# OthmanB/TAMCMC-C

Hardware: AMD Instinct MI355X
Metric: MCMC samples/sec (whole node), 1e5 nu-bins x 100 params x 20 tempered chains (higher is better)
Workload: dtype f64

## Files before the change

### tamcmc-c_amd/csrc/dev_sampler.hip

```cpp
#include <hip/hip_runtime.h>

#include <atomic>
#include <chrono>
#include <hip/hip_ext.h>

#include <cmath>
#include <cstdio>
#include <cstdlib>
#include <cstring>
#include <algorithm>
#include <type_traits>
#include <utility>
#include <vector>

#include "ctx.h"
#include "rgb_prestep.h"
#include "dev_sampler.h"
#include "kernels.h"
#include "loglike_tile.h"
#include "dev_unpack.h"
#include "fd_batch.h"
#include "mode_tables.h"
#include "rng.h"
#include "step_schedule.h"
// ... 189 lines not shown
    double *d_pr, *d_ex, *d_T;
    DCHK(I.dalloc(&d_pl, 11)); DCHK(I.dalloc(&d_idx, Nv)); DCHK(I.dalloc(&d_sw, Np));
    DCHK(I.dalloc(&d_pr, 4 * Np)); DCHK(I.dalloc(&d_ex, 10)); DCHK(I.dalloc(&d_T, C));
    DCHK(up(d_pl, in.plength, 11, st)); DCHK(up(d_idx, in.index_to_relax, Nv, st)); DCHK(up(d_sw, in.priors_switch, Np, st));
    DCHK(up(d_pr, in.priors, 4 * Np, st)); DCHK(up(d_ex, in.extra_priors, 10, st)); DCHK(up(d_T, in.Tcoefs, C, st));
    a.desc.plength = d_pl; a.index_to_relax = d_idx; a.desc.priors_switch = d_sw; a.desc.priors = d_pr; a.desc.extra = d_ex; a.Tcoefs = d_T;
    DCHK(I.dalloc(&a.vars_cur, 2 * C * Nv)); DCHK(I.dalloc(&a.params_cur, 2 * C * Np));
    DCHK(I.dalloc(&a.vars_prop, 2 * CD * Nv)); DCHK(I.dalloc(&a.params_prop, 2 * CD * Np));
    DCHK(I.dalloc(&a.logL_cur, 2 * C)); DCHK(I.dalloc(&a.logPr_cur, 2 * C)); DCHK(I.dalloc(&a.logPost_cur, 2 * C));
    DCHK(I.dalloc(&a.init_logL, C)); DCHK(I.dalloc(&a.logPr_prop, 2 * CD)); DCHK(I.dalloc(&a.status_prop, 2 * CD));
    DCHK(I.dalloc(&a.Pmove, C)); DCHK(I.dalloc(&a.moved, C)); DCHK(I.dalloc(&a.counters, 8 + C + 64));
    a.grad_cur = nullptr; a.gradP_cur = nullptr;
    if (I.use_drift) {
        DCHK(I.dalloc(&a.grad_cur, 2 * C * Nv)); DCHK(I.dalloc(&a.gradP_cur, 2 * C * Nv));
        DCHK(I.dalloc(&I.mala.grad_prop, C * Nv)); DCHK(I.dalloc(&I.mala.gradP_prop, C * Nv)); DCHK(I.dalloc(&I.mala.drift_cur, C * Nv));
        DCHK(I.dalloc(&I.mala.out, C * 5));
    }
    DCHK(I.dalloc(&a.lz, 2 * C * Nv)); DCHK(I.dalloc(&a.LT, C * Nv * Nv)); DCHK(I.dalloc(&a.cov, C * Nv * Nv)); DCHK(I.dalloc(&a.mu, C * Nv)); DCHK(I.dalloc(&a.sigma, C));
    DCHK(I.dalloc(&a.mults, CD * (size_t)a.desc.per + 1)); DCHK(I.dalloc(&a.pairs, 2 * CD)); DCHK(I.dalloc(&a.nh, CD)); DCHK(I.dalloc(&a.nn, CD));
    DCHK(I.dalloc(&a.noise, CD * (size_t)a.desc.stride));
    DCHK(hipMemsetAsync(a.counters, 0, (8 + C + 64) * sizeof(long), st));
    DCHK(hipMemsetAsync(a.moved, 0, C * sizeof(int), st));
    DCHK(hipMemsetAsync(a.Pmove, 0, C * sizeof(double), st));
    a.samples = nullptr; a.stats = nullptr;
    I.lds_base = (Np + 2 * Nv + 1) * sizeof(double) + unpack_lds_bytes() + 32;
    I.lds_adapt = (Nv * Nv + Nv) * sizeof(double);
    a.chol_in_lds = (I.lds_base + I.lds_adapt <= 150 * 1024) ? 1 : 0;
    if (!a.chol_in_lds) { DCHK(I.dalloc(&I.adapt_scratch, C * (Nv * Nv + Nv))); I.lds_adapt = 0; }
    if (I.lds_base + I.lds_adapt > 64 * 1024) {
        DCHK(hipFuncSetAttribute((const void *)k_iterate<true>, hipFuncAttributeMaxDynamicSharedMemorySize, (int)(I.lds_base + I.lds_adapt)));
        DCHK(hipFuncSetAttribute((const void *)k_iterate<false>, hipFuncAttributeMaxDynamicSharedMemorySize, (int)(I.lds_base + I.lds_adapt)));
    }
    mt::PolyTab *d_tab;
    DCHK(I.dalloc(&d_tab, 1));
    hipLaunchKernelGGL(k_fill_poly, dim3(1), dim3(64), 0, st, d_tab);
    DCHK(hipGetLastError());
    a.desc.poly = d_tab;
    for (int i = 0; i < 64; i++) { DCHK(hipEventCreate(&I.ev[i][0])); DCHK(hipEventCreate(&I.ev[i][1])); I.n_ev = i + 1; }
    for (int i = 0; i < 8; i++) { DCHK(hipEventCreate(&I.gev[i][0])); DCHK(hipEventCreate(&I.gev[i][1])); I.n_gev = i + 1; }
    {
        const int G = I.G;
        I.gst[0] = st;
        for (int g = 1; g < G; g++) DCHK(hipStreamCreateWithFlags(&I.gst[g], hipStreamNonBlocking));
        DCHK(hipEventCreateWithFlags(&I.ev_fork, hipEventDisableTiming));
        for (int g = 0; g < 4; g++) {
            DCHK(hipEventCreateWithFlags(&I.ev_kb[g], hipEventDisableTiming));
            DCHK(hipEventCreateWithFlags(&I.ev_ki[g], hipEventDisableTiming));
            DCHK(hipEventCreateWithFlags(&I.ev_join[g], hipEventDisableTiming));
        }
        I.ev_made = true;
    }
    {
        FusedArgs &f = I.f;
        f.NS = 2 * in.C + 8;
        {
            const int h = (int)(((long)in.C * 1) / 2);
            f.xsplit = (I.G == 2 && h >= 3 && in.C - h >= 3) ? h : in.C;
        }
        const size_t NS = (size_t)f.NS;
        DCHK(I.dalloc(&f.cand_vars, 3 * NS * Nv)); DCHK(I.dalloc(&f.cand_params, 3 * NS * Np)); DCHK(I.dalloc(&f.cand_logPr, 6 * NS));
        DCHK(I.dalloc(&f.cand_stP, 6 * NS)); DCHK(I.dalloc(&f.cand_stR, 3 * NS)); DCHK(I.dalloc(&f.cand_rej, 3 * NS));
        DCHK(I.dalloc(&f.mults, 3 * NS * (size_t)a.desc.per + 1)); DCHK(I.dalloc(&f.pairs, 6 * NS)); DCHK(I.dalloc(&f.nh, 3 * NS)); DCHK(I.dalloc(&f.nn, 3 * NS));
        DCHK(I.dalloc(&f.noise, 3 * NS * (size_t)a.desc.stride));
        DCHK(I.dalloc(&f.slot, 2 * C)); DCHK(I.dalloc(&f.prop_logPr, 2 * C)); DCHK(I.dalloc(&f.prop_st, 2 * C)); DCHK(I.dalloc(&f.quick, 2 * C * QN)); DCHK(I.dalloc(&f.lz, 2 * C * Nv));
        DCHK(I.dalloc(&f.qcount, 2));
        DCHK(hipMemsetAsync(f.qcount, 0, 2 * sizeof(unsigned long long), st));
        f.qmargin = 1e-11;
        DCHK(hipMemsetAsync(f.nn, 0, 3 * NS * sizeof(int), st));
        DCHK(hipMemsetAsync(f.cand_stP, 0, 6 * NS * sizeof(int), st));
        DCHK(hipMemsetAsync(f.cand_rej, 0, 3 * NS * sizeof(int), st));
        DCHK(hipMemsetAsync(f.cand_stR, 0, 3 * NS * sizeof(int), st));
        f.part = nullptr;
        f.psum = nullptr;
        f.bg = nullptr;
        const size_t role_lds = (Np + 2 * Nv + 1) * sizeof(double) + unpack_lds_bytes() + 32;
        I.fused_ok = !I.rgb && role_lds <= sizeof(tile::TileLds<tile::M_FAST_DIRECT, 64>);
    }
    DCHK(hipStreamSynchronize(st));
    return TAMCMC_OK;
}

int DevSampler::download_gradient(double *grad, double *grad_prior) {
    Impl &I = *impl;
    tamcmc_hip_ctx *c = I.ctx;
    if (!I.use_drift || !I.a.grad_cur || !I.grad_valid) return TAMCMC_ERR_BAD_ARG;
    DCHK(hipSetDevice(c->device));
    const size_t n = (size_t)I.a.C * I.a.Nv;
    DCHK(hipStreamSynchronize(c->stream));
    if (grad) DCHK(hipMemcpy(grad, I.a.grad_cur + (size_t)I.parity * n, n * sizeof(double), hipMemcpyDeviceToHost));
    if (grad_prior) DCHK(hipMemcpy(grad_prior, I.a.gradP_cur + (size_t)I.parity * n, n * sizeof(double), hipMemcpyDeviceToHost));
    return TAMCMC_OK;
}

int DevSampler::download_last_proposal(double *vars_prop, double *grad_prop) {
    Impl &I = *impl;
    tamcmc_hip_ctx *c = I.ctx;
    if (!I.use_drift) return TAMCMC_ERR_BAD_ARG;
    DCHK(hipSetDevice(c->device));
    const size_t n = (size_t)I.a.C * I.a.Nv;
    DCHK(hipStreamSynchronize(c->stream));
    if (vars_prop) DCHK(hipMemcpy(vars_prop, I.a.vars_prop, n * sizeof(double), hipMemcpyDeviceToHost));
    if (grad_prop) DCHK(hipMemcpy(grad_prop, I.mala.grad_prop, n * sizeof(double), hipMemcpyDeviceToHost));
    return TAMCMC_OK;
}

void DevSampler::info(long out[11]) const {
    const Impl &I = *impl;
    unsigned long long qc[2] = {0, 0};
    if (I.f.qcount && hipSetDevice(I.ctx->device) == hipSuccess) (void)hipMemcpy(qc, I.f.qcount, sizeof qc, hipMemcpyDeviceToHost);
    out[8] = I.n_stretch; out[9] = (long)qc[0]; out[10] = (long)qc[1];
// ... 129 lines not shown
static const bool g_call_timeline = getenv("TAMCMC_CALL_TIMELINE") != nullptr;
struct CallTimeline {
    std::chrono::steady_clock::time_point t[5];
    int n = 0;
    void mark() { if (g_call_timeline && n < 5) t[n++] = std::chrono::steady_clock::now(); }
    ~CallTimeline() {
        if (!g_call_timeline || n < 2) return;
        fprintf(stderr, "run() timeline (us):");
        for (int k = 1; k < n; k++) fprintf(stderr, " %.1f", std::chrono::duration<double, std::micro>(t[k] - t[k - 1]).count());
        fprintf(stderr, "\n");
    }
};

struct DevSampler::Impl::KernelTiming {
    Impl &I;
    tamcmc_hip_ctx *c;
    int used_ev = 0;
    std::vector<std::pair<int, long>> fused_ev;
    int g_used = 0;
    long g_launches = 0, g_iters = 0;
    double kernel_ms = 0;
    long n_launch = 0, n_eval = 0;
    bool stretch_timed = false;
    int fe = 0;
    long next_sample = 0;

    hipEvent_t *lockstep_pair(long k, long every) { return c->timing && k % every == 0 && used_ev < I.n_ev - 16 ? I.ev[used_ev++] : nullptr; }
    int drain_events(double launches_represented, long evals) {
        if (used_ev) {
            double tot = 0;
            for (int e = 0; e < used_ev; e++) {
                float ms = 0;
                DCHK(hipEventElapsedTime(&ms, I.ev[e][0], I.ev[e][1]));
                tot += ms;
            }
            kernel_ms += tot / used_ev * launches_represented;
            n_launch += (long)launches_represented;
            n_eval += evals;
        }
        used_ev = 0;
        return TAMCMC_OK;
    }
    void begin_fused(long len) {
        stretch_timed = c->timing && fused_ev.size() < 16;
        fe = I.n_ev - 1 - (int)fused_ev.size();
        next_sample = len >= 97 ? 48 : len / 2;
    }
    hipEvent_t *stretch_pair() { return stretch_timed ? I.ev[fe] : nullptr; }
    hipEvent_t *sampled_pair(long k) {
        if (!(stretch_timed && g_used < I.n_gev && k >= next_sample)) return nullptr;
        next_sample += 97;
        return I.gev[g_used++];
    }
    void end_fused(long len, bool split, long n_split) {
        if (!stretch_timed) return;
        if (!split) fused_ev.push_back({fe, len});
        else { g_launches += 2 * n_split + (len - n_split); g_iters += len; }
    }
    int total() {
        for (const auto &e : fused_ev) {
            float ms = 0;
            DCHK(hipEventElapsedTime(&ms, I.ev[e.first][0], I.ev[e.first][1]));
            kernel_ms += ms;
            n_launch += e.second;
            n_eval += e.second * (long)I.a.C;
        }
        if (g_launches > 0) {
            double tot = 0;
            for (int e = 0; e < g_used; e++) {
                float ms = 0;
                DCHK(hipEventElapsedTime(&ms, I.gev[e][0], I.gev[e][1]));
                tot += ms;
            }
            if (g_used > 0) {
                kernel_ms += tot / g_used * (double)g_launches;
                n_launch += g_launches;
                n_eval += g_iters * (long)I.a.C;
            }
        }
        c->kernel_ms += kernel_ms;
        c->launches += n_launch;
        c->evals += n_eval;
        return TAMCMC_OK;
    }
};

static hipError_t copy_records(double *samples, double *stats, const DevSamplerArgs &a, size_t n_iter, hipStream_t st) {
    const size_t C = (size_t)a.C, Nv = (size_t)a.Nv;
    hipError_t e = hipSuccess;
    if (samples) e = hipMemcpyAsync(samples, a.samples, n_iter * C * Nv * 8, hipMemcpyDeviceToHost, st);
    if (stats && e == hipSuccess) e = hipMemcpyAsync(stats, a.stats, n_iter * C * 3 * 8, hipMemcpyDeviceToHost, st);
    return e;
}

struct DevSampler::Impl::RunCall {
    Impl &I;
    tamcmc_hip_ctx *c;
    DevSamplerArgs &a;
    const long it0, n_iter;
    const char *learn;
    double *samples, *stats;
    hipStream_t st;
    CallTimeline &tl;
    KernelTiming T;
    DevSamplerArgs args;
    LoglikeArgs la[4], lf[3];
    int goff[5];
    double *zc_smp = nullptr, *zc_st = nullptr;
    bool use_fused = false;
    bool split_ok = false;
    int P;
    StepCtl sc{};
    int q = 0;
    bool s1_must_wait = false;
    bool s1_ahead = false;
    bool s1_open = false;

    RunCall(Impl &I_, CallTimeline &tl_, long it0_, long n_iter_, const char *learn_, double *samples_, double *stats_)
        : I(I_), c(I_.ctx), a(I_.a), it0(it0_), n_iter(n_iter_), learn(learn_), samples(samples_), stats(stats_), st(I_.ctx->stream),
          tl(tl_), T{I_, I_.ctx}, P(I_.parity) {}

    int prepare() {
        const size_t C = (size_t)a.C, Nv = (size_t)a.Nv;
        const int tb = tile_bins(c->wgs, c->K);
        a.ntiles = (a.desc.Nx + tb - 1) / tb;
        DCHK(c->d_part.reserve(C * (size_t)a.ntiles * 2));
        a.partials = c->d_part.p;
        a.tile_bins = tb;
        a.bg = nullptr;
        use_fused = I.fused_ok && c->step_scheme != 1 && c->wgs == 64 && (c->K == 4 || c->K == 8 || c->K == 16);
        I.f.qmargin = c->quick_decide == 1 ? (double)INFINITY : 1e-11;
        const size_t NS = (size_t)I.f.NS;
        I.f.bg = nullptr;
        if (c->precision == TAMCMC_PRECISION_FAST) {
            DCHK(c->d_bg.reserve(C * (size_t)a.ntiles * 8));
            a.bg = c->d_bg.p;
            if (use_fused) {
                DCHK(I.fused_bg.reserve(3 * NS * (size_t)a.ntiles * 8));
                I.f.bg = I.fused_bg.p;
            }
        }
        if (use_fused) {
            DCHK(I.fused_part.reserve(2 * C * (size_t)a.ntiles * 2));
            I.f.part = I.fused_part.p;
            DCHK(I.fused_psum.reserve(2 * C * (size_t)a.ntiles));
            I.f.psum = I.fused_psum.p;
        }
        split_ok = I.f.xsplit < a.C && c->step_scheme != 2 && (c->step_scheme == 3 || (long)a.C * a.ntiles >= 2500);
        auto grown = [](size_t need, size_t have, size_t unit) { const size_t floor_ = 256 * unit; return std::max(std::max(need, floor_), have * 2); };
        zc_smp = I.device_view(samples, (size_t)n_iter * C * Nv * 8);
        zc_st = I.device_view(stats, (size_t)n_iter * C * 3 * 8);
        if (samples && !zc_smp && I.smp_cap < (size_t)n_iter * C * Nv) {
            const size_t cap = grown((size_t)n_iter * C * Nv, I.smp_cap, C * Nv);
            DCHK(I.dalloc(&a.samples, cap));
            I.smp_cap = cap;
        }
        if (stats && !zc_st && I.stat_cap < (size_t)n_iter * C * 3) {
            const size_t cap = grown((size_t)n_iter * C * 3, I.stat_cap, C * 3);
            DCHK(I.dalloc(&a.stats, cap));
            I.stat_cap = cap;
        }
        args = a;
        args.samples = samples ? (zc_smp ? zc_smp : a.samples) : nullptr;
        args.stats = stats ? (zc_st ? zc_st : a.stats) : nullptr;
        const int G = I.G;
        for (int g = 0; g <= G; g++) goff[g] = (int)(((long)a.C * g) / G);
        auto fill_common = [&](LoglikeArgs &l, int B) {
            l.x = c->dx.p; l.y = c->dy.p; l.logx = c->dlogx.p; l.Nx = a.desc.Nx; l.B = B; l.ntiles = a.ntiles;
            l.x0 = a.desc.x_first; l.step = a.desc.step; l.noise_stride = a.desc.stride; l.model = nullptr; l.tile_rot = I.tile_rot;
        };
        for (int g = 0; g < G; g++) {
            LoglikeArgs &l = la[g];
            const int first = goff[g];
            fill_common(l, goff[g + 1] - goff[g]);
            l.mults = a.mults; l.offsets = a.pairs + 2 * first; l.noise = a.noise + (size_t)first * a.desc.stride;
            l.per = a.desc.per; l.slot0 = first;
            l.nharvey = a.nh + first; l.nnoise = a.nn + first; l.partials = a.partials + (size_t)first * a.ntiles * 2;
            l.bg_poly = a.bg ? a.bg + (size_t)first * a.ntiles * 8 : nullptr;
        }
        for (int e = 0; e < 3; e++) {
            LoglikeArgs &l = lf[e];
            const FusedArgs &f = I.f;
            fill_common(l, a.C);
            l.mults = f.mults + (size_t)e * NS * a.desc.per; l.offsets = f.pairs + (size_t)e * 2 * NS; l.noise = f.noise + (size_t)e * NS * a.desc.stride;
            l.nharvey = f.nh + (size_t)e * NS; l.nnoise = f.nn + (size_t)e * NS; l.partials = f.part;
            l.bg_poly = f.bg ? f.bg + (size_t)e * NS * a.ntiles * 8 : nullptr;
            l.per = a.desc.per; l.slot0 = 0;
        }
        return TAMCMC_OK;
    }

    int swap_pair_of(long it) const { return swap_pair(a.seed, a.C, a.dN_mixing, it, nullptr); }

    int run_lockstep(long ia, long ib) {
        const int G = I.G;
        const size_t C = (size_t)a.C;
        I.armed_it = -1;
        I.it_lockstep += ib - ia;
        if (G > 1) {
            DCHK(hipEventRecord(I.ev_fork, st));
            for (int g = 1; g < G; g++) DCHK(hipStreamWaitEvent(I.gst[g], I.ev_fork, 0));
// ... 37 lines not shown
            }
            P ^= 1;
            pending = 1;
            if (i < ib && I.rgb) {
                RgbDeviceTables R;
                R.mults = a.mults; R.pairs = a.pairs; R.nh = a.nh; R.nn = a.nn; R.noise = a.noise; R.stride = a.desc.stride;
                R.status = a.status_prop + (size_t)P * C;
                R.bg = a.bg; R.ntiles = a.ntiles; R.tile_bins = a.tile_bins;
                for (int g = 0; g < G; g++) {
                    int rc = rgb_device_stage(c, goff[g], goff[g + 1] - goff[g], I.rgb_bmax, g, a.desc.per, R, I.gst[g]);
                    if (rc) return rc;
                }
            }
            if (i < ib) {
                for (int g = 0; g < G; g++) {
                    hipEvent_t *pair = g == 0 ? T.lockstep_pair(i - ia, ev_every) : nullptr;
                    if (pair) DCHK(hipEventRecord(pair[0], I.gst[g]));
                    DCHK(launch_loglike(la[g], c->precision, c->wgs, c->K, false, I.gst[g]));
                    if (pair) DCHK(hipEventRecord(pair[1], I.gst[g]));
                }
            }
        }
        for (int g = 1; g < G; g++) {
            DCHK(hipEventRecord(I.ev_join[g], I.gst[g]));
            DCHK(hipStreamWaitEvent(st, I.ev_join[g], 0));
        }
        if (c->timing) {
            DCHK(hipStreamSynchronize(st));
            return T.drain_events((double)len * G, len * (long)a.C);
        }
        return TAMCMC_OK;
    }

    int sync_arg_image() {
        const size_t n1 = (sizeof(DevSamplerArgs) + 15) & ~(size_t)15, n2 = sizeof(FusedArgs);
        std::vector<unsigned char> img(n1 + n2, 0);
        std::memcpy(img.data(), &args, sizeof(DevSamplerArgs));
        std::memcpy(img.data() + n1, &I.f, sizeof(FusedArgs));
        if (!I.d_argcopy) DCHK(I.dalloc(&I.d_argcopy, n1 + n2));
        if (img != I.h_argcopy) {
            DCHK(hipMemcpyAsync(I.d_argcopy, img.data(), n1 + n2, hipMemcpyHostToDevice, st));
            DCHK(hipStreamSynchronize(st));
            I.h_argcopy = img;
            I.armed_it = -1;
        }
        sc.ga = (const DevSamplerArgs *)I.d_argcopy;
        sc.gf = (const FusedArgs *)(I.d_argcopy + n1);
        return TAMCMC_OK;
    }

    int fused_entry(long ia, bool *launched) {
        *launched = !(I.armed_it == it0 + ia && I.armed_q == q);
        if (!*launched) return TAMCMC_OK;
        const int nbr = 8 * I.f.NS;
        const int nlz2 = ((2 * a.C + 7) / 8) * 8;
        sc.it = it0 + ia; sc.rec = -1; sc.q = q; sc.flags = ST_LZ; sc.nbr = 0; sc.nlz = nlz2; sc.n_lz_live = 2 * a.C; sc.it_lz = it0 + ia; sc.q_lz = q;
        DCHK(launch_step(c->precision, c->K, nlz2, st, args, I.f, lf[0], sc));
        sc.flags = ST_ENTRY; sc.nbr = nbr; sc.nlz = 0; sc.n_lz_live = 0;
        DCHK(launch_step(c->precision, c->K, nbr, st, args, I.f, lf[0], sc));
        return TAMCMC_OK;
    }

    int launch_group(int first, int cnt, int A, int A_prev, long i, bool settled, hipStream_t stream, hipEvent_t *ev = nullptr) {
        const bool owns_pair = A >= first && A + 1 < first + cnt;
        const int ntiles_pad = ((a.ntiles + 7) / 8) * 8;
        sc.it = it0 + i; sc.rec = ((samples || stats) && !settled) ? i - 1 : (long)-1; sc.q = q;
        sc.flags = ST_L | ST_BR | ST_LZ | ST_COMMIT | (settled ? ST_FIRST : 0);
#ifdef TAMCMC_PROBE
        if (const char *ep = getenv("TAMCMC_PROBE_STEP")) {
            const int pm = atoi(ep);
            if (pm & 1) sc.flags &= ~ST_BR;
            if (pm & 2) sc.flags &= ~ST_COMMIT;
            if (pm & 4) sc.flags &= ~ST_LZ;
            if (pm & 8) sc.flags |= ST_FIRST;
            if (pm & 16) sc.flags &= ~ST_L;
        }
#endif
        sc.first = first; sc.cnt = cnt; sc.extra = owns_pair ? 1 : 0; sc.pairA = settled ? -1 : A_prev;
        sc.nbr = 8 * (2 * cnt + (owns_pair ? 4 : 0)); sc.nlz = ((2 * cnt + 7) / 8) * 8; sc.n_lz_live = cnt; sc.it_lz = it0 + i + 2; sc.q_lz = q;
        LoglikeArgs lq = lf[(it0 + i) % 3];
        lq.B = cnt;
        lq.partials = I.f.part + ((size_t)q * a.C + first) * a.ntiles * 2;
        DCHK(launch_step(c->precision, c->K, sc.nbr + sc.nlz + ntiles_pad * cnt, stream, args, I.f, lq, sc, ev ? ev[0] : nullptr, ev ? ev[1] : nullptr));
        return TAMCMC_OK;
    }

    int launch_close(int first, int cnt, long ib, hipStream_t stream) {
        sc.it = it0 + ib; sc.rec = (samples || stats) ? ib - 1 : (long)-1; sc.q = q;
        sc.flags = ST_COMMIT;
        sc.first = first; sc.cnt = cnt; sc.extra = 0;
        sc.nbr = 0; sc.nlz = ((cnt + 7) / 8) * 8; sc.n_lz_live = 0; sc.it_lz = 0; sc.q_lz = 0;
        DCHK(launch_step(c->precision, c->K, sc.nlz, stream, args, I.f, lf[0], sc));
        return TAMCMC_OK;
    }

    int s1_waits_for_st() {
        DCHK(hipEventRecord(I.ev_fork, st));
        DCHK(hipStreamWaitEvent(I.gst[1], I.ev_fork, 0));
        return TAMCMC_OK;
    }
    int st_waits_for_s1() {
        DCHK(hipEventRecord(I.ev_join[1], I.gst[1]));
        DCHK(hipStreamWaitEvent(st, I.ev_join[1], 0));
        return TAMCMC_OK;
    }

    int run_fused(long ia, long ib) {
        const long len = ib - ia;
        const int first1 = I.f.xsplit;
        hipStream_t s1 = I.gst[1];
        I.it_fused += len;
        I.n_stretch += 1;
        q = P;
        sc = StepCtl{};
        if (int rc = sync_arg_image()) return rc;
        sc.first = 0; sc.cnt = a.C; sc.extra = 1;
        bool entered;
        if (int rc = fused_entry(ia, &entered)) return rc;
        s1_must_wait = ia > 0 || entered;
        s1_ahead = false;
        T.begin_fused(len);
        if (!split_ok && T.stretch_pair()) DCHK(hipEventRecord(T.stretch_pair()[0], st));
        long n_split = 0;
        int A_prev = -1;
        for (long i = ia; i < ib; i++) {
            const int A = swap_pair_of(it0 + i);
            const bool settled = i == ia;
            if (!joint_launch(split_ok, first1, A, A_prev, settled)) {
                if (s1_must_wait) {
                    if (int rc = s1_waits_for_st()) return rc;
                    s1_must_wait = false;
                }
                if (int rc = launch_group(0, first1, A, A_prev, i, settled, st)) return rc;
                if (int rc = launch_group(first1, a.C - first1, A, A_prev, i, settled, s1, T.sampled_pair(i - ia))) return rc;
                s1_ahead = true;
                n_split++;
            } else {
                if (s1_ahead) {
                    if (int rc = st_waits_for_s1()) return rc;
                    s1_ahead = false;
                }
                if (int rc = launch_group(0, a.C, A, A_prev, i, settled, st)) return rc;
                s1_must_wait = true;
            }
            A_prev = A;
            q ^= 1;
        }
        if (s1_ahead) {
            if (int rc = launch_close(0, first1, ib, st)) return rc;
            if (int rc = launch_close(first1, a.C - first1, ib, s1)) return rc;
            if (ib >= n_iter) s1_open = true;
            else if (int rc = st_waits_for_s1()) return rc;
        } else if (int rc = launch_close(0, a.C, ib, st)) return rc;
        if (!split_ok && T.stretch_pair()) DCHK(hipEventRecord(T.stretch_pair()[1], st));
        T.end_fused(len, split_ok, n_split);
        P = q;
        I.armed_it = it0 + ib;
        I.armed_q = q;
        return TAMCMC_OK;
    }

    int finish() {
        I.parity = P;
        DCHK(hipGetLastError());
        tl.mark();
        double *const staged_smp = (samples && !zc_smp) ? samples : nullptr, *const staged_st = (stats && !zc_st) ? stats : nullptr;
        if (s1_open && (staged_smp || staged_st)) {
            if (int rc = st_waits_for_s1()) return rc;
            s1_open = false;
        }
        DCHK(copy_records(staged_smp, staged_st, a, (size_t)n_iter, st));
        const bool poll = g_running_calls.load(std::memory_order_relaxed) == 1;
        if (s1_open) DCHK(Impl::wait_stream(I.gst[1], poll));
        DCHK(Impl::wait_stream(st, poll));
        tl.mark();
        return T.total();
    }
};

int DevSampler::run(long it0, long n_iter, const char *learn, double *samples, double *stats) {
    RunningCall running_call;
    CallTimeline tl;
    tl.mark();
    Impl &I = *impl;
    tamcmc_hip_ctx *c = I.ctx;
    if (n_iter <= 0) return TAMCMC_OK;
    if (I.use_drift) return run_mala(it0, n_iter, learn, samples, stats);
    DCHK(hipSetDevice(c->device));
    Impl::RunCall r(I, tl, it0, n_iter, learn, samples, stats);
    if (int rc = r.prepare()) return rc;
    tl.mark();
    for (long i = 0, end = 0; i < n_iter; i = end) {
        bool is_fused;
        next_stretch(learn, n_iter, i, r.use_fused, &end, &is_fused);
        if (int rc = is_fused ? r.run_fused(i, end) : r.run_lockstep(i, end)) return rc;
    }
    return r.finish();
}

int DevSampler::run_mala(long it0, long n_iter, const char *learn, double *samples, double *stats) {
    Impl &I = *impl;
    tamcmc_hip_ctx *c = I.ctx;
    DevSamplerArgs &a = I.a;
    DCHK(hipSetDevice(c->device));
    hipStream_t st = c->stream;
    I.armed_it = -1;
    const size_t C = (size_t)a.C, Nv = (size_t)a.Nv, Np = (size_t)a.desc.Np;
    {
        FdBatch nb;
        int rc = nb.layout(c, I.model_id, I.prior_class, a.C, (int64_t)Np, I.h_plength.data(), a.Nv);
        if (rc) return rc;
        const bool need_bg = c->precision == TAMCMC_PRECISION_FAST && !I.fd_bg.p;
        if (nb.total_bytes != I.fd.total_bytes || nb.windowed != I.fd.windowed || nb.ntiles != I.fd.ntiles || !I.fd_block.p || need_bg) {
            I.fd = nb;
            rc = fd_ensure_poly(c);
            if (rc) return rc;
            DCHK(I.fd_block.reserve(nb.total_bytes));
            std::vector<unsigned char> hb(nb.in_bytes, 0);
            std::memcpy(hb.data() + nb.o_pr, I.h_priors.data(), 4 * Np * 8);
            std::memcpy(hb.data() + nb.o_ex, I.h_extra.data(), 10 * 8);
            std::memcpy(hb.data() + nb.o_sw, I.h_sw.data(), Np * 4);
            std::memcpy(hb.data() + nb.o_pl, I.h_plength.data(), 11 * 4);
            std::memcpy(hb.data() + nb.o_idx, I.h_idx.data(), Nv * 4);
            DCHK(hipMemcpyAsync(I.fd_block.p, hb.data(), nb.in_bytes, hipMemcpyHostToDevice, st));
            DCHK(hipStreamSynchronize(st));
            DCHK(I.fd_part.reserve(nb.nS * (size_t)nb.ntiles * 2));
// ... 91 lines not shown
```

### tamcmc-c_amd/csrc/dev_step_impl.h

```cpp

struct FusedArgs {
    int NS;
    int xsplit;
    double *cand_vars, *cand_params;
    double *cand_logPr;
    int *cand_rej;
    int *cand_stP, *cand_stR;
    tamcmc_multiplet *mults;
    int *pairs, *nh, *nn;
    double *noise;
    double *bg;
    int *slot;
    double *prop_logPr;
    int *prop_st;
    double *quick;
    double *part;
    double *psum;
    double *lz;
    double qmargin;
    unsigned long long *qcount;
};

constexpr int QN = 8;
constexpr int ST_L = 1, ST_BR = 2, ST_ENTRY = 4, ST_LZ = 8, ST_FIRST = 16, ST_COMMIT = 32;
// ... 33 lines not shown
        return s;
    }
    const int p = q ^ 1, ntiles = a.ntiles;
    const long itp = it - 1;
    int A = -1;
    double u = 0;
    if (is_swap_iter(a, itp)) A = swap_first(a, itp, &u);
    const bool in_pair = A >= 0 && (m == A || m == A + 1);
    const int j0 = in_pair ? A : m;
    const int jl = (in_pair && lane == 1) ? A + 1 : j0;
    const int ps = f.slot[p * C + jl] & 0xffff, st = f.prop_st[p * C + jl];
    const double pl = f.prop_logPr[p * C + jl], hL = a.logL_cur[p * C + jl], hP = a.logPr_cur[p * C + jl], hQ = a.logPost_cur[p * C + jl];
    const double Tj = a.Tcoefs[jl], il = a.init_logL[jl];
    const double *b0 = f.part + ((size_t)p * C + j0) * ntiles * 2;
    double S0, S1 = 0;
    if (ntiles <= TB) {
        double v1[TB / 64], v2[TB / 64], w1[TB / 64], w2[TB / 64];
#pragma unroll
        for (int k = 0; k < TB / 64; k++) {
            const int t = k * 64 + lane;
            const bool in = t < ntiles;
            v1[k] = in ? b0[2 * t] : 0.0;
            v2[k] = in ? b0[2 * t + 1] : 0.0;
            w1[k] = (in && in_pair) ? b0[2 * (ntiles + t)] : 0.0;
            w2[k] = (in && in_pair) ? b0[2 * (ntiles + t) + 1] : 0.0;
        }
#pragma unroll
        for (int k = 0; k < TB / 64; k++) { v1[k] = 0.0 + v1[k]; v2[k] = 0.0 + v2[k]; w1[k] = 0.0 + w1[k]; w2[k] = 0.0 + w2[k]; }
        S0 = wave_sum_in_order(v1, v2);
        if (in_pair) S1 = wave_sum_in_order(w1, w2);
    } else {
        S0 = wave_partial_sum(b0, ntiles);
        if (in_pair) S1 = wave_partial_sum(b0 + (size_t)ntiles * 2, ntiles);
    }
    AcceptOut o = mh_outcome(a, jl, itp, (in_pair && lane == 1) ? S1 : S0, pl, st, hL, hP, hQ, Tj, il);
    AcceptOut o0, o1;
    o0.acc = __shfl(o.acc, 0, 64); o0.r = __shfl(o.r, 0, 64); o0.logL = __shfl(o.logL, 0, 64); o0.logPr = __shfl(o.logPr, 0, 64);
    o0.logPost = __shfl(o.logPost, 0, 64);
    const int ps0 = __shfl(ps, 0, 64);
    Decided d;
    d.swap_first = -1; d.swapped = 0;
    if (!in_pair) {
        d.slot = 2 * m + o0.acc; d.src = m; d.src_acc = o0.acc; d.src_par = p; d.src_ps = ps0; d.r = o0.r; d.o = o0;
    } else {
        o1.acc = __shfl(o.acc, 1, 64); o1.r = __shfl(o.r, 1, 64); o1.logL = __shfl(o.logL, 1, 64); o1.logPr = __shfl(o.logPr, 1, 64);
        o1.logPost = __shfl(o.logPost, 1, 64);
        const int ps1 = __shfl(ps, 1, 64);
        const int accA = o0.acc, accB = o1.acc;
        const double rA = o0.r, rB = o1.r;
        const int swapped = resolve_swap(a, A, u, o0, o1);
        d.swap_first = A; d.swapped = swapped; d.src_par = p;
        const int B = A + 1;
        if (swapped) {
            if (m == A) { d.slot = 2 * C + (A >= f.xsplit ? 4 : 0) + accB; d.src = B; d.src_acc = accB; d.src_ps = ps1; d.r = rB; d.o = o0; }
            else { d.slot = 2 * C + (B >= f.xsplit ? 4 : 0) + 2 + accA; d.src = A; d.src_acc = accA; d.src_ps = ps0; d.r = rA; d.o = o1; }
        } else {
            if (m == A) { d.slot = 2 * A + accA; d.src = A; d.src_acc = accA; d.src_ps = ps0; d.r = rA; d.o = o0; }
            else { d.slot = 2 * B + accB; d.src = B; d.src_acc = accB; d.src_ps = ps1; d.r = rB; d.o = o1; }
        }
    }
    if (out && lane == 0) *out = d;
    return d.slot;
}

__device__ __attribute__((noinline)) void commit_chain(const DevSamplerArgs *ga, const FusedArgs *gf, int m, long it, int q, int settled, long rec,
                                                       int tiles, Decided *dec) {
    const int slot = decide(ga, gf, m, it, q, settled, dec);
    __syncthreads();
    const ConstArgs &a = *(const ConstArgs *)uniform_ptr(ga);
    const ConstFused &f = *(const ConstFused *)uniform_ptr(gf);
    const int lane = threadIdx.x, C = a.C, Nv = a.Nv, Np = a.desc.Np;
    const Decided d = *dec;
    if (lane == 0) {
        const size_t gs = (size_t)(it % 3) * f.NS + slot;
        const int stP0 = f.cand_stP[2 * gs], stP1 = f.cand_stP[2 * gs + 1], stR = f.cand_stR[gs];
        const double lp = f.cand_rej[gs] ? -INFINITY : f.cand_logPr[2 * gs] + f.cand_logPr[2 * gs + 1];
        const int stm = stP0 != TAMCMC_OK ? stP0 : (stP1 != TAMCMC_OK ? stP1 : stR);
        f.prop_logPr[q * C + m] = lp;
        f.prop_st[q * C + m] = stm;
        double *w = f.quick + ((size_t)q * C + m) * QN;
        const double Tm = a.Tcoefs[m];
        double Sstar = 0, ok = -1;
        double u, u1;
        rng_uniform2(a.seed, RNG_ACCEPT, (uint32_t)m, (uint64_t)it, 0, u, u1);
        if (stm == TAMCMC_OK && !(lp == -INFINITY || isnan(lp))) {
            const double cur = settled ? a.logPost_cur[q * C + m] : d.o.logPost;
            Sstar = -((log(u) - lp + cur) * Tm) / (double)a.pl;
            if (isfinite(Sstar)) ok = 1;
        } else if (u > 0.0) ok = 2;
        w[0] = Sstar; w[1] = ok; w[2] = -(double)a.pl / Tm; w[3] = settled ? a.logL_cur[q * C + m] : d.o.logL;
        double lus = 0, k1 = 0, k2 = 0;
        if (is_swap_iter(a, it)) {
            double us;
            if (swap_first(a, it, &us) == m) {
                const double TB = a.Tcoefs[m + 1];
                lus = log(us); k1 = Tm / TB - 1.0; k2 = TB / Tm - 1.0;
            }
        }
        w[4] = lus; w[5] = k1; w[6] = k2; w[7] = (double)slot;
    }
    if (settled) return;
    const double *sv, *sp;
    if (d.src_acc) {
        const size_t gp = (size_t)((it - 1) % 3) * f.NS + d.src_ps;
        sv = f.cand_vars + gp * Nv;
        sp = f.cand_params + gp * Np;
    } else {
        sv = a.vars_cur + ((size_t)d.src_par * C + d.src) * Nv;
// ... 41 lines not shown
            s0 += v[k]; a0 += fabs(v[k]);
            if (PAIR) { s1 += w[k]; a1 += fabs(w[k]); }
        }
    }
#pragma unroll
    for (int off = 32; off >= 1; off >>= 1) {
        s0 += __shfl_xor(s0, off, 64); a0 += __shfl_xor(a0, off, 64);
        if (PAIR) { s1 += __shfl_xor(s1, off, 64); a1 += __shfl_xor(a1, off, 64); }
    }
}
__device__ __forceinline__ int quick_decide_core(const DevSamplerArgs *ga, const FusedArgs *gf, int m, int q, int pairA, Decided *out) {
    const ConstArgs &a = *(const ConstArgs *)uniform_ptr(ga);
    const ConstFused &f = *(const ConstFused *)uniform_ptr(gf);
    const int lane = threadIdx.x & 63, C = a.C;
    const int p = q ^ 1, n = a.ntiles;
    const bool in_pair = pairA >= 0 && (m == pairA || m == pairA + 1);
    const int j0 = in_pair ? pairA : m;
    const double *c0 = f.psum + ((size_t)p * C + j0) * n;
    const double *r0 = f.quick + ((size_t)p * C + j0) * QN;
    double rec, s0 = 0, a0 = 0, s1 = 0, a1 = 0;
    if (in_pair) {
        rec = lane < 2 * QN ? r0[lane] : 0.0;
        quick_sums<true>(c0, n, lane, s0, a0, s1, a1);
    } else {
        rec = lane < QN ? r0[lane] : 0.0;
        quick_sums<false>(c0, n, lane, s0, a0, s1, a1);
    }
    const double St0 = __shfl(rec, 0, 64), ok0 = __shfl(rec, 1, 64);
    const int ps0 = (int)__shfl(rec, 7, 64);
    const double mg = f.qmargin;
    int acc0 = 0;
    if (ok0 == 2.0) { s0 = 0; a0 = 0; }
    else if (ok0 > 0 && fabs(s0 - St0) > mg * (a0 + fabs(St0))) acc0 = s0 < St0 ? 1 : 0;
    else return -1;
    Decided d;
    d.swap_first = -1; d.swapped = 0; d.src_par = p; d.r = 0;
    d.o.acc = 0; d.o.r = 0; d.o.logL = 0; d.o.logPr = 0; d.o.logPost = 0;
    if (!in_pair) { d.slot = 2 * m + acc0; d.src = m; d.src_acc = acc0; d.src_ps = ps0; }
    else {
        const double St1 = __shfl(rec, QN, 64), ok1 = __shfl(rec, QN + 1, 64);
        const int ps1 = (int)__shfl(rec, QN + 7, 64);
        int acc1 = 0;
        if (ok1 == 2.0) { s1 = 0; a1 = 0; }
        else if (ok1 > 0 && fabs(s1 - St1) > mg * (a1 + fabs(St1))) acc1 = s1 < St1 ? 1 : 0;
        else return -1;
        const double c0 = __shfl(rec, 2, 64), c1 = __shfl(rec, QN + 2, 64);
        const double LA = acc0 ? c0 * s0 : __shfl(rec, 3, 64), LB = acc1 ? c1 * s1 : __shfl(rec, QN + 3, 64);
        const double lus = __shfl(rec, 4, 64), x = LA * __shfl(rec, 5, 64) + LB * __shfl(rec, 6, 64);
        if (!(fabs(x - lus) > mg * (fabs(c0) * a0 + fabs(c1) * a1 + fabs(LA) + fabs(LB)))) return -1;
        const int swapped = x > lus ? 1 : 0;
        const int A = pairA, B = pairA + 1;
        d.swap_first = A; d.swapped = swapped;
        if (swapped) {
            if (m == A) { d.slot = 2 * C + (A >= f.xsplit ? 4 : 0) + acc1; d.src = B; d.src_acc = acc1; d.src_ps = ps1; }
            else { d.slot = 2 * C + (B >= f.xsplit ? 4 : 0) + 2 + acc0; d.src = A; d.src_acc = acc0; d.src_ps = ps0; }
        } else {
            if (m == A) { d.slot = 2 * A + acc0; d.src = A; d.src_acc = acc0; d.src_ps = ps0; }
            else { d.slot = 2 * B + acc1; d.src = B; d.src_acc = acc1; d.src_ps = ps1; }
        }
    }
    if (out && lane == 0) *out = d;
    return d.slot;
}
__device__ __attribute__((noinline)) int quick_decide_leaf(const DevSamplerArgs *ga, const FusedArgs *gf, int m, int q, int pairA, Decided *out) {
    return quick_decide_core(ga, gf, m, q, pairA, out);
}

__device__ __forceinline__ int quick_decide(const DevSamplerArgs *ga, const FusedArgs *gf, int m, long it, int q, int settled, int pairA,
                                            Decided *out) {
    if (settled) return decide(ga, gf, m, it, q, 1, out);
    const int s = quick_decide_leaf(ga, gf, m, q, pairA, out);
    return s >= 0 ? s : decide(ga, gf, m, it, q, 0, out);
}

__device__ __attribute__((noinline)) int decide_counted(const DevSamplerArgs *ga, const FusedArgs *gf, int m, long it, int q, int tile) {
    if (tile == 0 && (threadIdx.x & 63) == 0) atomicAdd(((const ConstFused *)uniform_ptr(gf))->qcount, 1ull);
    return decide(ga, gf, m, it, q, 0, nullptr);
}

struct StepTiles {
    const DevSamplerArgs *ga;
    const FusedArgs *gf;
    long it;
    int q, first, settled, pairA;
    static constexpr bool coherent_partials = false;
    static constexpr bool early_loads = true;
    __device__ __forceinline__ tile::SlotWords head(const LoglikeArgs &a, int b, int tile) const {
        const int m = first + b;
        if (settled) return tile::slot_words(a, decide(ga, gf, m, it, q, 1, nullptr));
        const bool lone = a.per > 0 && !(pairA >= 0 && (m == pairA || m == pairA + 1));
        tile::SlotWords w0{}, w1{};
        if (lone) { w0 = tile::slot_words(a, 2 * m); w1 = tile::slot_words(a, 2 * m + 1); }
        int s = quick_decide_core(ga, gf, m, q, pairA, nullptr);
        if (s < 0) s = decide_counted(ga, gf, m, it, q, tile);
        if (lone && (s >> 1) == m) return (s & 1) ? w1 : w0;
        return tile::slot_words(a, s);
    }
    __device__ __forceinline__ void store_sums(int b, int tile, double s0, double s1) const {
        const ConstArgs &a = *(const ConstArgs *)uniform_ptr(ga);
        const ConstFused &f = *(const ConstFused *)uniform_ptr(gf);
        f.psum[((size_t)q * a.C + first + b) * a.ntiles + tile] = s0 + s1;
    }
    __device__ __forceinline__ void operator()(int, int, int) const {}
};

__device__ __attribute__((noinline)) void role_prior(const DevSamplerArgs *ga, const FusedArgs *gf, size_t gs, int h, const double *s_vars,
                                                     const double *s_params, const UnpackLds *Up) {
    const DevSamplerArgs &a = *ga;
// ... 36 lines not shown
#ifdef TAMCMC_PROBE
    __shared__ long ps_[8];
    wg_unpack(a.desc, s_params, U, slot, T, true, false, false, true, ps_);
    __syncthreads();
    if (threadIdx.x == 0 && (int)(gs % f.NS) == 2) {
        long *w = a.counters + 8 + a.C + 8 + 4; w[0] += ps_[1] - ps_[0]; w[1] += ps_[2] - ps_[1];
        long *v = a.counters + 8 + a.C + 32; v[0] += ps_[5] - ps_[4]; v[1] += ps_[6] - ps_[5]; v[2] += ps_[7] - ps_[6]; v[3] += 1;
    }
#else
    wg_unpack(a.desc, s_params, U, slot, T, true, false, false, true);
#endif
    if (threadIdx.x == 0) f.cand_stR[gs] = *U.status;
}
__device__ __attribute__((noinline)) void role_background(const DevSamplerArgs *ga, const FusedArgs *gf, int q_dst, int slot, int role,
                                                          const double *s_params, const UnpackLds *Up) {
    const DevSamplerArgs &a = *ga;
    const FusedArgs &f = *gf;
    const UnpackLds U = *Up;
    if (!f.bg) return;
    if (threadIdx.x == 0) mt::shared_scalars_base(a.desc.model_id, s_params, a.desc.plength, *U.S);
    __syncthreads();
    TablePtrs T = candidate_tables(a, f, q_dst);
    T.bg = f.bg + (size_t)q_dst * f.NS * a.ntiles * bg::NH;
    const int quarter = (a.ntiles + 3) / 4, k = role - 3;
    wg_bg_tiles(a.desc, s_params, U.S, slot, T, 0, 64, k * quarter, (k + 1) * quarter);
}

__device__ __attribute__((noinline)) void lz_normals(const DevSamplerArgs *ga, long itn, int m, double *s_z) {
    normals_into(*ga, m, itn, s_z);
}
__device__ __attribute__((noinline)) void lz_rows(const DevSamplerArgs *ga, const FusedArgs *gf, int q_dst, int m, const double *s_z) {
    Lz_rows_wave(*ga, m, s_z, gf->lz + ((size_t)q_dst * ga->C + m) * ga->Nv);
}
__device__ __forceinline__ void lz_block(const DevSamplerArgs *ga, const FusedArgs *gf, long itn, int q_dst, int m, unsigned char *lds) {
    double *s_z = (double *)lds;
    lz_normals(ga, itn, m, s_z);
    __syncthreads();
    lz_rows(ga, gf, q_dst, m, s_z);
}

__device__ void candidate_role(const DevSamplerArgs &a, const FusedArgs &f, const DevSamplerArgs *ga, const FusedArgs *gf, long itn, int q_src,
                               int q_dst, int slot, int role, bool entry, int settled, int pairA, unsigned char *lds, Decided *dec) {
    if (role > 6) return;
    const int C = a.C, Nv = a.Nv, Np = a.desc.Np, tid = threadIdx.x;
    const int e_dst = (int)(itn % 3);
    int m, src, on_prop;
    if (slot < 2 * C) { m = slot >> 1; src = m; on_prop = slot & 1; }
    else {
        if (entry || !is_swap_iter(a, itn - 1)) return;
        const int A = swap_first(a, itn - 1, nullptr), e = slot - 2 * C;
        m = (e < 2) ? A : A + 1;
        src = (e < 2) ? A + 1 : A;
        on_prop = e & 1;
        slot += (m >= f.xsplit) ? 4 : 0;
    }
    if (entry && on_prop) return;
    if (entry && role == 0 && tid == 0) f.slot[q_src * C + m] = 2 * m;
#ifdef TAMCMC_PROBE
    long pt[6];
    pt[0] = (long)wall_clock64();
#define RSTAMP(k) pt[k] = (long)wall_clock64()
#else
#define RSTAMP(k)
#endif
    double *s_params = (double *)lds;
    double *s_vars = s_params + Np;
    double *s_z = s_vars + Nv;
    const UnpackLds U = carve_unpack_lds((unsigned char *)(s_z + Nv + 1));
    __shared__ UnpackLds s_U;
    if (tid == 0) s_U = U;
    const double *bv, *bp;
    if (entry) {
        bv = a.vars_cur + ((size_t)q_src * C + src) * Nv;
        bp = a.params_cur + ((size_t)q_src * C + src) * Np;
    } else {
        const int ps = quick_decide(ga, gf, src, itn - 1, q_src, settled, pairA, dec);
        __syncthreads();
        const Decided d = *dec;
        if (on_prop) {
            const size_t gp = (size_t)((itn - 1) % 3) * f.NS + ps;
            bv = f.cand_vars + gp * Nv;
            bp = f.cand_params + gp * Np;
        } else if (d.src_acc) {
            const size_t gp = (size_t)((itn - 2) % 3) * f.NS + d.src_ps;
            bv = f.cand_vars + gp * Nv;
            bp = f.cand_params + gp * Np;
        } else {
            bv = a.vars_cur + ((size_t)d.src_par * C + d.src) * Nv;
            bp = a.params_cur + ((size_t)d.src_par * C + d.src) * Np;
        }
    }
    RSTAMP(1);
    const double *lz = f.lz + ((size_t)q_dst * C + m) * Nv;
    constexpr int PW = (int)(sizeof(mt::PolyTab) / sizeof(double));
    if (Nv <= 128 && Np <= 128 && PW <= 256) {
        double r_v[2], r_z[2], r_p[2], r_t[4];
        int r_i[2];
#pragma unroll
        for (int e = 0; e < 2; e++) {
            const int i = tid + 64 * e;
            r_v[e] = i < Nv ? bv[i] : 0.0; r_z[e] = i < Nv ? lz[i] : 0.0; r_i[e] = i < Nv ? a.index_to_relax[i] : 0;
            r_p[e] = i < Np ? bp[i] : 0.0;
        }
#pragma unroll
        for (int e = 0; e < 4; e++) { const int i = tid + 64 * e; r_t[e] = i < PW ? ((const double *)a.desc.poly)[i] : 0.0; }
#pragma unroll
        for (int e = 0; e < 2; e++) { const int i = tid + 64 * e; if (i < Np) s_params[i] = r_p[e]; }
// ... 104 lines not shown
```

### tamcmc-c_amd/csrc/step_schedule.h

```cpp
#pragma once
#include "rng.h"

namespace tamcmc {


#define TAMCMC_HD_FLAT TAMCMC_HD __attribute__((always_inline))

TAMCMC_HD_FLAT bool is_swap_iteration(int C, long dN_mixing, long it) { return dN_mixing > 0 && (it % dN_mixing == 0) && it != 0 && C > 1; }

TAMCMC_HD_FLAT int swap_draw(uint64_t seed, int C, long it, double *u_out) {
    double u, u2;
    rng_uniform2(seed, RNG_SWAP, 0, (uint64_t)it, 0, u, u2);
    int A = (int)(u2 * (double)(C - 1));
    if (A > C - 2) A = C - 2;
    if (u_out) *u_out = u;
    return A;
}

TAMCMC_HD_FLAT int swap_pair(uint64_t seed, int C, long dN_mixing, long it, double *u_out) {
    return is_swap_iteration(C, dN_mixing, it) ? swap_draw(seed, C, it, u_out) : -1;
}


TAMCMC_HD int group_of(int chain, const int *goff, int G) {
    int g = 0;
    while (g + 1 < G && chain >= goff[g + 1]) g++;
    return g;
}


constexpr long MIN_FUSED = 3;

TAMCMC_HD long quiet_end(const char *learn, long n_iter, long from) {
    long q = from;
    while (q < n_iter && !(learn && learn[q])) q++;
    return q;
}

TAMCMC_HD void next_stretch(const char *learn, long n_iter, long i, bool use_fused, long *end, bool *is_fused) {
    const long jn = quiet_end(learn, n_iter, i);
    if (use_fused && jn - i >= MIN_FUSED) {
        *end = jn;
        *is_fused = true;
        return;
    }
    long k = i;
    for (;;) {
        const long q = quiet_end(learn, n_iter, k);
        if (use_fused && q - k >= MIN_FUSED && k > i) break;
        k = q;
        while (k < n_iter && learn && learn[k]) k++;
        if (k >= n_iter) break;
    }
    *end = k;
    *is_fused = false;
}


TAMCMC_HD bool straddles(bool split_ok, int xsplit, int A) { return split_ok && A == xsplit - 1; }

TAMCMC_HD bool joint_launch(bool split_ok, int xsplit, int A, int A_prev, bool first) {
    return !split_ok || straddles(split_ok, xsplit, A) || (!first && straddles(split_ok, xsplit, A_prev));
}

}
```

Before: 48790.

## Split straddling swap iterations across three streams instead of joint launch

When a swap pair straddles the split between the two chain groups, the whole ensemble used to be launched jointly on the main stream, which serialised both groups. A third stream now runs the small band of chains around the boundary, while the lower and upper groups keep running on their own streams. Cross-stream dependencies are tracked per chain through events. Cross-swap candidate slots are re-indexed per chain, so the candidate buffers grow to 4*C. This adds event record/wait overhead and more complex sync logic, with some risk of subtle ordering bugs.

```diff
diff --git a/tamcmc-c_amd/csrc/dev_sampler.hip b/tamcmc-c_amd/csrc/dev_sampler.hip
--- a/tamcmc-c_amd/csrc/dev_sampler.hip
+++ b/tamcmc-c_amd/csrc/dev_sampler.hip
@@ -265,10 +265,11 @@
     }
     {
         FusedArgs &f = I.f;
-        f.NS = 2 * in.C + 8;
+        f.NS = 4 * in.C;
         {
             const int h = (int)(((long)in.C * 1) / 2);
             f.xsplit = (I.G == 2 && h >= 3 && in.C - h >= 3) ? h : in.C;
+            if (f.xsplit < in.C) DCHK(hipStreamCreateWithFlags(&I.gst[2], hipStreamNonBlocking));
         }
         const size_t NS = (size_t)f.NS;
         DCHK(I.dalloc(&f.cand_vars, 3 * NS * Nv)); DCHK(I.dalloc(&f.cand_params, 3 * NS * Np)); DCHK(I.dalloc(&f.cand_logPr, 6 * NS));
@@ -504,10 +505,10 @@
         next_sample += 97;
         return I.gev[g_used++];
     }
-    void end_fused(long len, bool split, long n_split) {
+    void end_fused(long len, bool split, long n_launches) {
         if (!stretch_timed) return;
         if (!split) fused_ev.push_back({fe, len});
-        else { g_launches += 2 * n_split + (len - n_split); g_iters += len; }
+        else { g_launches += n_launches; g_iters += len; }
     }
     int total() {
         for (const auto &e : fused_ev) {
@@ -564,9 +565,11 @@
     int P;
     StepCtl sc{};
     int q = 0;
-    bool s1_must_wait = false;
-    bool s1_ahead = false;
-    bool s1_open = false;
+    bool pair_ok = false;
+    bool must_wait[3] = {false, false, false};
+    bool ahead[3] = {false, false, false};
+    bool open[3] = {false, false, false};
+    int last_stream[TAMCMC_MAX_CHAINS];
 
     RunCall(Impl &I_, CallTimeline &tl_, long it0_, long n_iter_, const char *learn_, double *samples_, double *stats_)
         : I(I_), c(I_.ctx), a(I_.a), it0(it0_), n_iter(n_iter_), learn(learn_), samples(samples_), stats(stats_), st(I_.ctx->stream),
@@ -599,6 +602,7 @@
             I.f.psum = I.fused_psum.p;
         }
         split_ok = I.f.xsplit < a.C && c->step_scheme != 2 && (c->step_scheme == 3 || (long)a.C * a.ntiles >= 2500);
+        pair_ok = split_ok && I.gst[2] != nullptr;
         auto grown = [](size_t need, size_t have, size_t unit) { const size_t floor_ = 256 * unit; return std::max(std::max(need, floor_), have * 2); };
         zc_smp = I.device_view(samples, (size_t)n_iter * C * Nv * 8);
         zc_st = I.device_view(stats, (size_t)n_iter * C * 3 * 8);
@@ -742,7 +746,7 @@
     int fused_entry(long ia, bool *launched) {
         *launched = !(I.armed_it == it0 + ia && I.armed_q == q);
         if (!*launched) return TAMCMC_OK;
-        const int nbr = 8 * I.f.NS;
+        const int nbr = 8 * 2 * a.C;
         const int nlz2 = ((2 * a.C + 7) / 8) * 8;
         sc.it = it0 + ia; sc.rec = -1; sc.q = q; sc.flags = ST_LZ; sc.nbr = 0; sc.nlz = nlz2; sc.n_lz_live = 2 * a.C; sc.it_lz = it0 + ia; sc.q_lz = q;
         DCHK(launch_step(c->precision, c->K, nlz2, st, args, I.f, lf[0], sc));
@@ -784,66 +788,93 @@
         return TAMCMC_OK;
     }
 
-    int s1_waits_for_st() {
+    hipStream_t stream_of(int k) const { return k == 0 ? st : I.gst[k]; }
+    int stream_waits_for_st(int k) {
         DCHK(hipEventRecord(I.ev_fork, st));
-        DCHK(hipStreamWaitEvent(I.gst[1], I.ev_fork, 0));
-        return TAMCMC_OK;
-    }
-    int st_waits_for_s1() {
-        DCHK(hipEventRecord(I.ev_join[1], I.gst[1]));
-        DCHK(hipStreamWaitEvent(st, I.ev_join[1], 0));
+        DCHK(hipStreamWaitEvent(I.gst[k], I.ev_fork, 0));
+        return TAMCMC_OK;
+    }
+    int st_waits_for_stream(int k) {
+        DCHK(hipEventRecord(I.ev_join[k], I.gst[k]));
+        DCHK(hipStreamWaitEvent(st, I.ev_join[k], 0));
+        return TAMCMC_OK;
+    }
+
+    int launch_iteration(long i, long ia, long ib, int A, int A_prev, long *n_launches) {
+        const bool settled = i == ia, close = i == ib;
+        const StepLaunches L = step_launches(step_plan(split_ok, pair_ok, a.C, I.f.xsplit, A, A_prev, settled), a.C);
+        unsigned hopped = 0;
+        for (int l = 0; l < L.n && L.n > 1; l++) {
+            const int k = L.stream[l];
+            if (k == 0 || !must_wait[k]) continue;
+            if (int rc = stream_waits_for_st(k)) return rc;
+            must_wait[k] = false;
+            hopped |= 1u << k;
+        }
+        unsigned deps_of[3], recorded = 0;
+        for (int l = 0; l < L.n; l++) {
+            const int k = L.stream[l];
+            deps_of[l] = step_dependencies(last_stream, L.first[l], L.cnt[l], k);
+            if (L.n == 1) deps_of[l] = 0;
+            else if (hopped & (1u << k)) deps_of[l] &= ~1u;
+            for (int j = 0; j < 3; j++)
+                if ((deps_of[l] & ~recorded) & (1u << j)) DCHK(hipEventRecord(I.ev_kb[j], stream_of(j)));
+            recorded |= deps_of[l];
+        }
+        for (int l = 0; l < L.n; l++) {
+            const int k = L.stream[l];
+            const unsigned deps = deps_of[l];
+            if (L.n == 1) {
+                for (int j = 1; j < 3; j++)
+                    if (ahead[j]) {
+                        if (int rc = st_waits_for_stream(j)) return rc;
+                        ahead[j] = false;
+                    }
+                must_wait[1] = must_wait[2] = true;
+            } else if (k > 0) ahead[k] = true;
+            for (int j = 0; j < 3; j++)
+                if (deps & (1u << j)) DCHK(hipStreamWaitEvent(stream_of(k), I.ev_kb[j], 0));
+            if (close) {
+                if (int rc = launch_close(L.first[l], L.cnt[l], ib, stream_of(k))) return rc;
+            } else if (int rc = launch_group(L.first[l], L.cnt[l], A, A_prev, i, settled, stream_of(k), k == 1 ? T.sampled_pair(i - ia) : nullptr))
+                return rc;
+        }
+        if (!close) *n_launches += L.n;
         return TAMCMC_OK;
     }
 
     int run_fused(long ia, long ib) {
         const long len = ib - ia;
-        const int first1 = I.f.xsplit;
-        hipStream_t s1 = I.gst[1];
         I.it_fused += len;
         I.n_stretch += 1;
         q = P;
         sc = StepCtl{};
         if (int rc = sync_arg_image()) return rc;
-        sc.first = 0; sc.cnt = a.C; sc.extra = 1;
+        sc.first = 0; sc.cnt = a.C; sc.extra = 0;
         bool entered;
         if (int rc = fused_entry(ia, &entered)) return rc;
-        s1_must_wait = ia > 0 || entered;
-        s1_ahead = false;
+        must_wait[1] = must_wait[2] = ia > 0 || entered;
+        ahead[1] = ahead[2] = false;
+        for (int m = 0; m < a.C; m++) last_stream[m] = -1;
         T.begin_fused(len);
         if (!split_ok && T.stretch_pair()) DCHK(hipEventRecord(T.stretch_pair()[0], st));
-        long n_split = 0;
+        long n_launches = 0;
         int A_prev = -1;
         for (long i = ia; i < ib; i++) {
             const int A = swap_pair_of(it0 + i);
-            const bool settled = i == ia;
-            if (!joint_launch(split_ok, first1, A, A_prev, settled)) {
-                if (s1_must_wait) {
-                    if (int rc = s1_waits_for_st()) return rc;
-                    s1_must_wait = false;
-                }
-                if (int rc = launch_group(0, first1, A, A_prev, i, settled, st)) return rc;
-                if (int rc = launch_group(first1, a.C - first1, A, A_prev, i, settled, s1, T.sampled_pair(i - ia))) return rc;
-                s1_ahead = true;
-                n_split++;
-            } else {
-                if (s1_ahead) {
-                    if (int rc = st_waits_for_s1()) return rc;
-                    s1_ahead = false;
-                }
-                if (int rc = launch_group(0, a.C, A, A_prev, i, settled, st)) return rc;
-                s1_must_wait = true;
-            }
+            if (int rc = launch_iteration(i, ia, ib, A, A_prev, &n_launches)) return rc;
             A_prev = A;
             q ^= 1;
         }
-        if (s1_ahead) {
-            if (int rc = launch_close(0, first1, ib, st)) return rc;
-            if (int rc = launch_close(first1, a.C - first1, ib, s1)) return rc;
-            if (ib >= n_iter) s1_open = true;
-            else if (int rc = st_waits_for_s1()) return rc;
-        } else if (int rc = launch_close(0, a.C, ib, st)) return rc;
+        if (int rc = launch_iteration(ib, ia, ib, -1, A_prev, &n_launches)) return rc;
+        for (int k = 1; k < 3; k++) {
+            if (!ahead[k]) continue;
+            if (ib >= n_iter) open[k] = true;
+            else if (int rc = st_waits_for_stream(k)) return rc;
+            ahead[k] = false;
+        }
         if (!split_ok && T.stretch_pair()) DCHK(hipEventRecord(T.stretch_pair()[1], st));
-        T.end_fused(len, split_ok, n_split);
+        T.end_fused(len, split_ok, n_launches);
         P = q;
         I.armed_it = it0 + ib;
         I.armed_q = q;
@@ -855,13 +886,15 @@
         DCHK(hipGetLastError());
         tl.mark();
         double *const staged_smp = (samples && !zc_smp) ? samples : nullptr, *const staged_st = (stats && !zc_st) ? stats : nullptr;
-        if (s1_open && (staged_smp || staged_st)) {
-            if (int rc = st_waits_for_s1()) return rc;
-            s1_open = false;
-        }
+        for (int k = 1; k < 3; k++)
+            if (open[k] && (staged_smp || staged_st)) {
+                if (int rc = st_waits_for_stream(k)) return rc;
+                open[k] = false;
+            }
         DCHK(copy_records(staged_smp, staged_st, a, (size_t)n_iter, st));
         const bool poll = g_running_calls.load(std::memory_order_relaxed) == 1;
-        if (s1_open) DCHK(Impl::wait_stream(I.gst[1], poll));
+        for (int k = 1; k < 3; k++)
+            if (open[k]) DCHK(Impl::wait_stream(I.gst[k], poll));
         DCHK(Impl::wait_stream(st, poll));
         tl.mark();
         return T.total();
diff --git a/tamcmc-c_amd/csrc/dev_step_impl.h b/tamcmc-c_amd/csrc/dev_step_impl.h
--- a/tamcmc-c_amd/csrc/dev_step_impl.h
+++ b/tamcmc-c_amd/csrc/dev_step_impl.h
@@ -109,8 +109,8 @@
         d.swap_first = A; d.swapped = swapped; d.src_par = p;
         const int B = A + 1;
         if (swapped) {
-            if (m == A) { d.slot = 2 * C + (A >= f.xsplit ? 4 : 0) + accB; d.src = B; d.src_acc = accB; d.src_ps = ps1; d.r = rB; d.o = o0; }
-            else { d.slot = 2 * C + (B >= f.xsplit ? 4 : 0) + 2 + accA; d.src = A; d.src_acc = accA; d.src_ps = ps0; d.r = rA; d.o = o1; }
+            if (m == A) { d.slot = cross_slot(C, A, accB); d.src = B; d.src_acc = accB; d.src_ps = ps1; d.r = rB; d.o = o0; }
+            else { d.slot = cross_slot(C, B, accA); d.src = A; d.src_acc = accA; d.src_ps = ps0; d.r = rA; d.o = o1; }
         } else {
             if (m == A) { d.slot = 2 * A + accA; d.src = A; d.src_acc = accA; d.src_ps = ps0; d.r = rA; d.o = o0; }
             else { d.slot = 2 * B + accB; d.src = B; d.src_acc = accB; d.src_ps = ps1; d.r = rB; d.o = o1; }
@@ -258,8 +258,8 @@
         const int A = pairA, B = pairA + 1;
         d.swap_first = A; d.swapped = swapped;
         if (swapped) {
-            if (m == A) { d.slot = 2 * C + (A >= f.xsplit ? 4 : 0) + acc1; d.src = B; d.src_acc = acc1; d.src_ps = ps1; }
-            else { d.slot = 2 * C + (B >= f.xsplit ? 4 : 0) + 2 + acc0; d.src = A; d.src_acc = acc0; d.src_ps = ps0; }
+            if (m == A) { d.slot = cross_slot(C, A, acc1); d.src = B; d.src_acc = acc1; d.src_ps = ps1; }
+            else { d.slot = cross_slot(C, B, acc0); d.src = A; d.src_acc = acc0; d.src_ps = ps0; }
         } else {
             if (m == A) { d.slot = 2 * A + acc0; d.src = A; d.src_acc = acc0; d.src_ps = ps0; }
             else { d.slot = 2 * B + acc1; d.src = B; d.src_acc = acc1; d.src_ps = ps1; }
@@ -402,7 +402,7 @@
         m = (e < 2) ? A : A + 1;
         src = (e < 2) ? A + 1 : A;
         on_prop = e & 1;
-        slot += (m >= f.xsplit) ? 4 : 0;
+        slot = cross_slot(C, m, on_prop);
     }
     if (entry && on_prop) return;
     if (entry && role == 0 && tid == 0) f.slot[q_src * C + m] = 2 * m;
diff --git a/tamcmc-c_amd/csrc/step_schedule.h b/tamcmc-c_amd/csrc/step_schedule.h
--- a/tamcmc-c_amd/csrc/step_schedule.h
+++ b/tamcmc-c_amd/csrc/step_schedule.h
@@ -63,4 +63,45 @@
     return !split_ok || straddles(split_ok, xsplit, A) || (!first && straddles(split_ok, xsplit, A_prev));
 }
 
+
+struct StepPlan {
+    bool joint;
+    int lo, hi;
+};
+TAMCMC_HD StepPlan step_plan(bool split_ok, bool pair_ok, int C, int xsplit, int A, int A_prev, bool first) {
+    StepPlan p;
+    p.joint = joint_launch(split_ok, xsplit, A, A_prev, first);
+    p.lo = p.hi = xsplit;
+    if (!split_ok || !p.joint) { p.joint = !split_ok; return p; }
+    const int Q = first ? -1 : A_prev;
+    p.lo = xsplit - 1; p.hi = xsplit + 1;
+    const int other = straddles(split_ok, xsplit, A) ? Q : A;
+    if (other >= 0 && other + 1 == p.lo) p.lo = other;
+    if (other >= 0 && other == p.hi - 1) p.hi = other + 2;
+    p.joint = !pair_ok || p.lo < 1 || p.hi > C - 1;
+    return p;
 }
+struct StepLaunches {
+    int n, first[3], cnt[3], stream[3];
+};
+TAMCMC_HD StepLaunches step_launches(const StepPlan &p, int C) {
+    StepLaunches L;
+    L.n = 0;
+    if (p.joint) { L.first[0] = 0; L.cnt[0] = C; L.stream[0] = 0; L.n = 1; return L; }
+    if (p.hi > p.lo) { L.first[L.n] = p.lo; L.cnt[L.n] = p.hi - p.lo; L.stream[L.n] = 2; L.n++; }
+    L.first[L.n] = 0; L.cnt[L.n] = p.lo; L.stream[L.n] = 0; L.n++;
+    L.first[L.n] = p.hi; L.cnt[L.n] = C - p.hi; L.stream[L.n] = 1; L.n++;
+    return L;
+}
+TAMCMC_HD unsigned step_dependencies(int *last, int first, int cnt, int stream) {
+    unsigned deps = 0;
+    for (int m = first; m < first + cnt; m++) {
+        if (last[m] >= 0 && last[m] != stream) deps |= 1u << last[m];
+        last[m] = stream;
+    }
+    return deps;
+}
+
+TAMCMC_HD_FLAT int cross_slot(int C, int m, int on_prop) { return 2 * C + 2 * m + on_prop; }
+
+}
```

After: 46430. 0.952x the previous value.
